# SunJiamei/LRP-ImageCaptioning

Measured on AMD Instinct MI355X. Metric: LRP heatmaps/sec (per predicted token) VGG16+adaptive-attn, 224x224, higher is better.
Workload: dtype bf16x3; 1 GPU; batch=32 synthetic 224x224 per GPU, VGG16 + adaptive-attention, LRP per-token heat-maps, 10 words/caption, V=10000 (BASELINE configs[1]); parallelism=image-sharded x1, RCCL weight broadcast, reverse_walk_precision=bf16x3, handles_per_gpu=2

## Files before the change

include/lrp_hip.h:

```cpp
#ifndef LRP_HIP_H
#define LRP_HIP_H

#include <stddef.h>
#include <stdint.h>

#ifdef __cplusplus
extern "C" {
#endif

#define LRP_ABI_VERSION 8

enum {
  LRP_OK = 0,
  LRP_ERR_INVALID = -1,
  LRP_ERR_STATE = -2,
  LRP_ERR_HIP = -3,
  LRP_ERR_NOMEM = -4,
  LRP_ERR_RANGE = -5,
  LRP_ERR_UNSUPPORTED = -6
};

enum { LRP_DEC_ADAPTIVE = 0,
       LRP_DEC_GRIDTD = 1 };

enum { LRP_EXPLAIN_SEQUENCE = 0,
       LRP_EXPLAIN_SINGLE_STEP = 1  };

enum { LRP_ENC_VGG = 0, LRP_ENC_RESNET = 1 };

#define LRP_MAX_CONV 32

typedef struct lrp_config {
  int32_t abi_version;
// ... 50 lines not shown

int lrp_decoder_gen_begin(lrp_handle* h, int32_t B, void* stream);
int lrp_decoder_gen_step(lrp_handle* h, int32_t B, const int32_t* parent_host, const int32_t* word_host, int32_t step,
                         double* logits_dev, void* stream);
int lrp_op_log_softmax_topk(const double* logits_dev, int32_t rows, int32_t V, int32_t k, int32_t* ids_dev,
                            double* logp_dev, void* stream);

int lrp_decoder_gradient(lrp_handle* h, int32_t n, const int32_t* img_idx_host, const int32_t* t_host,
                         float* d_feat_dev, double* r_words_dev, void* stream);
enum { LRP_WALK_LRP = 0, LRP_WALK_GRADIENT = 1, LRP_WALK_INPUT_X_GRADIENT = 2, LRP_WALK_GUIDED_BACKPROP = 3 };
int lrp_cnn_walk(lrp_handle* h, int32_t n, const int32_t* img_idx_host, const float* head_dev, float* out_dev,
                 int32_t walk, void* stream);

enum { LRP_PREC_FP32 = 0, LRP_PREC_BF16X3 = 1, LRP_PREC_BF16X3_FAST = 2, LRP_PREC_F16X2 = 3 };
int lrp_set_precision(lrp_handle* h, int32_t mode);
int lrp_set_fast_layers(lrp_handle* h, int64_t mask);

int lrp_profile_enable(lrp_handle* h, int32_t on);
int lrp_profile_query(lrp_handle* h, int64_t* n_launches, double* total_ms, double* total_flop);
int lrp_profile_records(lrp_handle* h, int32_t cap, double* ms_out, double* flop_out, int32_t* n_out);

int64_t lrp_workspace_bytes(const lrp_handle* h);

enum { LRP_CONV_SPLIT_BF16 = 0x100 };
int lrp_op_conv(const float* in_dev, const float* w_hwio_host, const float* bias_host,
                const float* aux_dev, float* out_dev, int32_t NB, int32_t H, int32_t W,
                int32_t Cin, int32_t Cout, int32_t taps, int32_t mode, void* stream);

int lrp_op_conv_pool_sparse(const float* sc_dev, const unsigned char* pos_dev, const float* w_hwio_host, const float* gate_dev,
                            float* out_dev, int32_t NB, int32_t Hp, int32_t Wp, int32_t Cin, int32_t Cout, int32_t reps, void* stream);

int lrp_op_epsilon_dense(const float* x_dev, const float* W_host, const float* R_dev, float* out_dev,
                         int32_t N, int32_t Din, int32_t Dout, float epsilon, void* stream);
int lrp_op_batchnorm_lrp(const float* x_dev, const float* gamma_dev, const float* beta_dev, const float* mean_dev,
                         const float* var_dev, float bn_eps, const float* R_dev, float* out_dev, int64_t n,
                         int32_t C, void* stream);
int lrp_op_add_lrp(const float* a_dev, const float* b_dev, const float* R_dev, float* Ra_dev, float* Rb_dev,
                   int64_t n, void* stream);

int lrp_op_avgpool_lrp(const float* x_dev, const float* R_dev, float* out_dev, int32_t NB, int32_t H, int32_t W,
                       int32_t C, int32_t k, void* stream);

int lrp_heatmap_render(const float* R_img_dev, const float* lut_dev, float* rgb_dev, int32_t n, int32_t npix, int32_t C,
                       float gamma, void* stream);

int lrp_preprocess_images(const uint8_t* rgb_dev, float* out_dev, int32_t NB, int32_t H0, int32_t W0, int32_t H,
                          int32_t W, void* stream);
// ... 57 lines not shown
```

lrp-imagecaptioning_amd/_capi.py:

```python
import ctypes as C
import os

HERE = os.path.dirname(os.path.abspath(__file__))
LIB_PATH = os.path.join(HERE, "liblrp_hip.so")

LRP_ABI_VERSION = 8
LRP_OK, LRP_ERR_INVALID, LRP_ERR_STATE, LRP_ERR_HIP, LRP_ERR_NOMEM, LRP_ERR_RANGE, LRP_ERR_UNSUPPORTED = 0, -1, -2, -3, -4, -5, -6
LRP_DEC_ADAPTIVE, LRP_DEC_GRIDTD = 0, 1
LRP_ENC_VGG, LRP_ENC_RESNET = 0, 1
LRP_EXPLAIN_SEQUENCE, LRP_EXPLAIN_SINGLE_STEP = 0, 1
LRP_PREC_FP32, LRP_PREC_BF16X3, LRP_PREC_BF16X3_FAST, LRP_PREC_F16X2 = 0, 1, 2, 3
LRP_MAX_CONV = 32
LRP_TRAIN_FP32, LRP_TRAIN_BF16 = 0, 1
LRP_EPI_BIAS_RELU, LRP_EPI_BIAS, LRP_EPI_MUL, LRP_EPI_MUL_UP2, LRP_EPI_FWD_DUAL, LRP_EPI_STORE, LRP_EPI_IMG_STENCIL = range(7)
LRP_OPND_FP32, LRP_OPND_BF16X3, LRP_OPND_F16X2 = 0, 1, 2
LRP_FORM_PLAIN, LRP_FORM_SMALL, LRP_FORM_HALO, LRP_FORM_BREG, LRP_FORM_POOL, LRP_FORM_IMG = range(6)
LRP_PLAN_FRAG, LRP_PLAN_JOIN, LRP_PLAN_DUAL_IL, LRP_PLAN_GMASK, LRP_PLAN_UP2_SRC, LRP_PLAN_IMG_PART, LRP_PLAN_POOL_GC = 1, 2, 4, 8, 16, 32, 64


class LrpConfig(C.Structure):
    _fields_ = [
        ("abi_version", C.c_int32), ("device", C.c_int32), ("decoder", C.c_int32),
        ("img_h", C.c_int32), ("img_w", C.c_int32), ("n_conv", C.c_int32),
        ("conv_cin", C.c_int32 * LRP_MAX_CONV), ("conv_cout", C.c_int32 * LRP_MAX_CONV),
        ("conv_pool_after", C.c_int32 * LRP_MAX_CONV), ("conv_name", (C.c_char * 32) * LRP_MAX_CONV),
        ("L", C.c_int32), ("D", C.c_int32), ("H", C.c_int32), ("E", C.c_int32), ("V", C.c_int32),
        ("max_images", C.c_int32), ("max_tokens", C.c_int32), ("max_caption_len", C.c_int32),
        ("sos_id", C.c_int32), ("eos_id", C.c_int32),
        ("encoder", C.c_int32), ("resnet_stem", C.c_int32), ("resnet_n_stacks", C.c_int32),
# ... 99 lines not shown
```

lrp-imagecaptioning_amd/csrc/conv_igemm.h:

```cpp
#pragma once
#include <hip/hip_runtime.h>
#include <stdint.h>
#include <stdlib.h>
#include <string.h>
#include <algorithm>
#include <vector>

#include "common.h"

namespace lrp {

typedef float f32x4 __attribute__((ext_vector_type(4)));
typedef float f32x16 __attribute__((ext_vector_type(16)));
typedef unsigned int u32x4 __attribute__((ext_vector_type(4)));
typedef __bf16 bf16x8 __attribute__((ext_vector_type(8)));
typedef _Float16 f16x8 __attribute__((ext_vector_type(8)));

enum ConvPrec { PREC_FP32 = 0, PREC_BF16X3 = 1, PREC_F16X2 = 2 };

__device__ __forceinline__ void split8h_store(const float* r, float* dst) {
  f16x8 hi, lo;
#pragma unroll
  for (int q = 0; q < 8; ++q) {
    hi[q] = (_Float16)r[q];
// ... 40 lines not shown
  ~TileOrder() {
    if (dev) (void)hipFree(dev);
    if (pinned) (void)hipHostFree(pinned);
    if (ev) (void)hipEventDestroy(ev);
  }
};

struct ConvArgs {
  const float* in;
  const float* wpk;
  const float* wpk_frag;
  int NB, H, W, Cin, CinP;
  int N;
  int taps;
  int M;
  int m_tiles, n_tiles;
  const float* bias;
  float* out;
  float* out2;
  const float* aux;
  const int* row2img;
  int split;
  int out_plain;
  int tiles_x, tiles_y, img_mode;
  const float* ximg;
  const float* addend;
  const float* gate_src;
  const float* join;
  const float* join_gate;
  const float* gate2;
  float* out2s;
  int gate_binary, relu_out;
  int dual_norelu;
  int dual_il, dual_gate;
  const float* bn_gamma; const float* bn_beta; const float* bn_mean; const float* bn_var;
  float bn_eps; int bn_relu;
  int tw, th, hrows, cols_t, nyh;
  const int* tile_map;
  TileOrder* order;
  const int* row2img_host;
  const float* tok_fac;
  unsigned* tok_max_out;
  const float* in_unscale;
  unsigned* act_max_out;
  float* pairs_out;
  const float* pairs_scale;
// ... 794 lines not shown
        for (int c = 0; c < 3; ++c) { pos[c] *= sc; neg[c] *= sc; }
      }
      const float* xv = a.ximg + ((size_t)img * HW + (size_t)y * a.W + x) * 3;
      float* ov = a.out + ((size_t)pn * HW + (size_t)y * a.W + x) * 3;
#pragma unroll
      for (int c = 0; c < 3; ++c) {
        if (a.img_mode == 0) ov[c] = xv[c] >= 0.f ? xv[c] * pos[c] : xv[c] * neg[c];
        else if (a.img_mode == 1) ov[c] = pos[c] + neg[c];
        else ov[c] = xv[c] * (pos[c] + neg[c]);
      }
    }
    return;
  } else if constexpr (EPI != EPI_STORE) {
    constexpr int NH = (BM * BN + 2 * STAGE - 1) / (2 * STAGE);
    constexpr int RH = BM / NH;
    static_assert(BM % NH == 0 && RH % (TM * 32) == 0 && RH * BN <= 2 * STAGE, "slab must hold whole wave tiles");
    float* Cs = smem;
    constexpr bool SPLIT_OUT = SPLIT && (EPI == EPI_MUL || EPI == EPI_MUL_UP2);
    constexpr int CW = SPLIT_OUT ? 8 : 4;
    constexpr int C4 = BN / CW, RPP = NT / C4;
    const int c4 = tid % C4, rin = tid / C4;
    const int col = n0 + c4 * CW;
    const int tn0 = m0 / HW, tp0 = m0 - tn0 * HW;
    const float invw = 1.0f / (float)a.W;
    auto locate = [&](int lr, int& row, int& n, int& h, int& w) -> bool {
      if constexpr (HALO) {
        int ty, tx;
        divmod(lr, a.tw, inv_tw, ty, tx);
        const int Y = Y0 + ty;
        w = x0 + tx;
        if (lr >= a.th * a.tw || Y >= yend || w >= a.W) return false;
        divmod(Y, a.H, inv_H, n, h);
        row = Y * a.W + w;
        return true;
      } else {
        row = m0 + lr;
        if (row >= a.M) return false;
        if constexpr (EPI == EPI_MUL || EPI == EPI_MUL_UP2) {
          n = tn0;
          int pix = tp0 + lr;
          while (pix >= HW) { pix -= HW; ++n; }
          h = (int)(((float)pix + 0.5f) * invw);
          w = pix - h * a.W;
          if (w < 0) { --h; w += a.W; } else if (w >= a.W) { ++h; w -= a.W; }
        }
        return true;
// ... 307 lines not shown
                }
              };
#pragma unroll
              for (int ps = 0; ps < RING - 1; ++ps) issue(ps);
              const bool plain = SPLIT_OUT && a.out_plain;
#pragma unroll
              for (int ps = 0; ps < NPf; ++ps) {
                if (ps + RING - 1 < NPf) issue(ps + RING - 1);
                int row, n_, h_, w_;
                if (locate(hf * RH + rin + ps * RPP, row, n_, h_, w_)) {
                  const int ll = rin + ps * RPP;
                  float v[CW];
#pragma unroll
                  for (int q4 = 0; q4 < CW / 4; ++q4)
                    *reinterpret_cast<f32x4*>(v + 4 * q4) = *reinterpret_cast<const f32x4*>(Cs + ll * BN + c4 * CW + 4 * q4);
#pragma unroll
                  for (int q = 0; q < UPf; ++q) {
                    float r[CW];
#pragma unroll
                    for (int q4 = 0; q4 < CW / 4; ++q4)
#pragma unroll
                      for (int e = 0; e < 4; ++e) r[4 * q4 + e] = v[4 * q4 + e] * gq[ps % RING][q][q4][e];
                    float* dst = EPI == EPI_MUL
                                     ? a.out + (size_t)row * a.N + col
                                     : a.out + (((size_t)n_ * H2f + 2 * h_ + (q >> 1)) * W2f + 2 * w_ + (q & 1)) * a.N + col;
                    if constexpr (SPLIT_OUT) {
                      if (plain) {
                        *reinterpret_cast<f32x4*>(dst) = *reinterpret_cast<const f32x4*>(r);
                        *reinterpret_cast<f32x4*>(dst + 4) = *reinterpret_cast<const f32x4*>(r + 4);
                      } else {
                        split8_store(r, dst);
                      }
                    } else {
                      *reinterpret_cast<f32x4*>(dst) = *reinterpret_cast<const f32x4*>(r);
                    }
                  }
                }
              }
              continue;
            }
          }
          constexpr int NP = RH / RPP;
          constexpr int UPN = EPI == EPI_MUL_UP2 ? 4 : 1;
          const int W2 = 2 * a.W, H2 = 2 * a.H;
          int rowv[NP], nv[NP], hv[NP], wv[NP], imgv[NP];
          bool okv[NP];
#pragma unroll
// ... 73 lines not shown
                *reinterpret_cast<f32x4*>(v + 4 * q4) = *reinterpret_cast<const f32x4*>(Cs + ll * BN + c4 * CW + 4 * q4);
#pragma unroll
              for (int q = 0; q < UPN; ++q) {
                float r[CW];
#pragma unroll
                for (int q4 = 0; q4 < CW / 4; ++q4) {
                  f32x4 g = cur.g[q][q4];
                  if (a.gate_binary) {
#pragma unroll
                    for (int e = 0; e < 4; ++e) g[e] = g[e] != 0.f ? 1.f : 0.f;
                  }
#pragma unroll
                  for (int e = 0; e < 4; ++e) {
                    float pr = v[4 * q4 + e] * g[e];
                    if (tail) pr += cur.jn[q4][e] * cur.jg[q4][e];
                    if constexpr (PREC == PREC_F16X2) {
                      pr *= fac16;
                      lmax = max(lmax, __float_as_uint(fabsf(pr)));
                    }
                    r[4 * q4 + e] = a.relu_out ? fmaxf(pr, 0.f) : pr;
                  }
                }
                float* dst = EPI == EPI_MUL
                                 ? a.out + (size_t)rowv[ps] * a.N + col
                                 : a.out + (((size_t)nv[ps] * H2 + 2 * hv[ps] + (q >> 1)) * W2 + 2 * wv[ps] + (q & 1)) * a.N + col;
                if constexpr (SPLIT_OUT) {
                  if (a.out_plain) {
                    *reinterpret_cast<f32x4*>(dst) = *reinterpret_cast<const f32x4*>(r);
                    *reinterpret_cast<f32x4*>(dst + 4) = *reinterpret_cast<const f32x4*>(r + 4);
                  } else if constexpr (PREC == PREC_F16X2) {
                    split8h_store(r, dst);
                  } else {
                    split8_store(r, dst);
                  }
                } else {
                  *reinterpret_cast<f32x4*>(dst) = *reinterpret_cast<const f32x4*>(r);
                }
                if (head2) {
                  float r2[CW];
#pragma unroll
                  for (int q4 = 0; q4 < CW / 4; ++q4)
#pragma unroll
                    for (int e = 0; e < 4; ++e) r2[4 * q4 + e] = r[4 * q4 + e] * cur.g2[q4][e];
                  float* d2 = a.out2s + (size_t)rowv[ps] * a.N + col;
                  if constexpr (SPLIT_OUT) {
                    split8_store(r2, d2);
                  } else {
// ... 258 lines not shown
  a.epi_generic = p.epi_generic;
}

template <int PREC>
inline hipError_t conv_launch_img(ConvArgs a, hipStream_t st) {
  if (!a.ximg || (PREC == PREC_F16X2 && !a.tok_fac)) return hipErrorInvalidValue;
  const ConvPlan p = conv_plan(conv_ask(EPI_IMG_STENCIL, PREC, 7, false, a));
  if (!p.ok) return hipErrorInvalidValue;
  if (a.NB <= 0) return hipSuccess;
  conv_apply_plan(p, a);
  a.tiles_x = (a.W + IMG_TILE - 1) / IMG_TILE;
  a.tiles_y = (a.H + IMG_TILE - 1) / IMG_TILE;
  hipLaunchKernelGGL((conv_igemm_kernel<4, 1, 2, 2, EPI_IMG_STENCIL, PREC>), dim3(a.m_tiles), dim3(p.threads), 0, st, a);
  return hipGetLastError();
}

template <int EPI, int PREC, int TERMS = 7, bool GMASK = false>
inline hipError_t conv_launch_epi(ConvArgs a, hipStream_t st) {
  static_assert(!GMASK || (EPI == EPI_MUL && PREC == PREC_FP32), "byte-mask gates: exact fp32 EPI_MUL only");
  constexpr bool MUL = EPI == EPI_MUL || EPI == EPI_MUL_UP2, FWD = EPI == EPI_BIAS || EPI == EPI_BIAS_RELU || EPI == EPI_FWD_DUAL;
  if (GMASK && (a.out2s || a.gate_none)) return hipErrorInvalidValue;
  if (PREC == PREC_F16X2 && MUL && (!a.tok_fac || !a.tok_max_out || a.out_plain)) return hipErrorInvalidValue;
  if (PREC == PREC_F16X2 && FWD && !a.in_unscale) return hipErrorInvalidValue;
  const ConvPlan p = conv_plan(conv_ask(EPI, PREC, TERMS, GMASK, a));
  if (!p.ok) return hipErrorInvalidValue;
  if (p.M <= 0 || a.N <= 0) return hipSuccess;
  if (a.pool_gc && (!a.pairs_out || !a.pool_pos)) return hipErrorInvalidValue;
  if (a.img_part && !a.img_w) return hipErrorInvalidValue;
  if (a.up2_src && (!a.up2_pairs || !a.up2_gpos)) return hipErrorInvalidValue;
  conv_apply_plan(p, a);
  const dim3 grid(p.m_tiles * p.n_tiles), block(p.threads);
  if constexpr (PREC != PREC_FP32 && (MUL || FWD)) {
    if (p.form == FORM_BREG || p.form == FORM_HALO || p.form == FORM_POOL) {
      if constexpr (MUL) {
        a.tile_map = conv_tile_order(a, st);
        if (p.form == FORM_BREG) {
          hipLaunchKernelGGL((conv_igemm_kernel<2, 2, 2, 1, EPI, PREC, true, true, TERMS>), grid, block, 0, st, a);
          return hipGetLastError();
        }
      }
      if (p.BM == 256)
        hipLaunchKernelGGL((conv_igemm_kernel<2, 4, 4, 2, EPI, PREC, true, false, TERMS>), grid, block, 0, st, a);
      else if (p.BN == 128)
        hipLaunchKernelGGL((conv_igemm_kernel<2, 2, 2, 2, EPI, PREC, true, false, TERMS>), grid, block, 0, st, a);
      else
        hipLaunchKernelGGL((conv_igemm_kernel<2, 2, 2, 1, EPI, PREC, true, false, TERMS>), grid, block, 0, st, a);
// ... 73 lines not shown
```

lrp-imagecaptioning_amd/csrc/conv_sparse.h:

```cpp
#pragma once
#include "cnn_kernels.h"
#include "conv_igemm.h"

namespace lrp {

typedef __bf16 bf16x16 __attribute__((ext_vector_type(16)));
typedef unsigned u32x2 __attribute__((ext_vector_type(2)));

struct SparseArgs {
  const float* sc;
  const unsigned* idxp;
  const float* wsp;
  const float* gate;
  float* out;
  const int* row2img;
  int NB, Hp, Wp, C, N;
  int cols_t, m_tiles, n_tiles;
  int out_plain;
  int diag;
};

constexpr int SP_TW = 14, SP_PITCH = SP_TW + 2;
constexpr int SP_BPACK = 32768, SP_NSTAGE = 4;

// ... 55 lines not shown
      const unsigned mh = px ^ qxm, mv = py ^ qym;
      const unsigned nmh = mh ^ 0x01010101u, nmv = mv ^ 0x01010101u;
      word[0][d] = P | ((P ^ 0x01010101u) << 2);
      word[1][d] = py | nmh | (nmh << 1);
      word[2][d] = (0x02020202u | ((mh & mv) ^ 0x01010101u)) << 2;
      word[3][d] = (px & mv) | (nmv << 1) | 0x0C0C0C0Cu;
    }
    unsigned h0[4], h1[4];
#pragma unroll
    for (int pl = 0; pl < 4; ++pl) {
      const unsigned t0 = word[pl][0] | (word[pl][0] >> 4), t1 = word[pl][1] | (word[pl][1] >> 4);
      h0[pl] = (t0 & 0xFFu) | (((t0 >> 16) & 0xFFu) << 8);
      h1[pl] = (t1 & 0xFFu) | (((t1 >> 16) & 0xFFu) << 8);
    }
    const u32x4 iw = {h0[0] | (h0[1] << 16), h0[2] | (h0[3] << 16), h1[0] | (h1[1] << 16), h1[2] | (h1[3] << 16)};
    const int spw = C >> 3;
    const size_t win = set / spw;
    const int sw = (int)(set - win * spw), chunk = sw >> 1, s2 = sw & 1;
    const size_t img = win / HW, pix = win - img * HW;
    reinterpret_cast<u32x4*>(idxp)[((((img * 4 + q) * (C >> 4) + chunk) * HW + pix) << 1) + s2] = iw;
  }
}

__global__ __launch_bounds__(256) void conv_sparse_pairs_kernel(const float* __restrict__ sc, float* __restrict__ scp, size_t n_sets, int HW, int C) {
  for (size_t i = (size_t)blockIdx.x * 256 + threadIdx.x; i < n_sets; i += (size_t)gridDim.x * 256) {
    float v[8];
    *reinterpret_cast<f32x4*>(v) = *reinterpret_cast<const f32x4*>(sc + i * 8);
    *reinterpret_cast<f32x4*>(v + 4) = *reinterpret_cast<const f32x4*>(sc + i * 8 + 4);
    const int spw = C >> 3;
    const size_t win = i / spw;
    const int sw = (int)(i - win * spw), chunk = sw >> 1, s2 = sw & 1;
    const size_t n = win / HW, pix = win - n * HW;
    split8_store(v, scp + ((((n * (C >> 4) + chunk) * HW + pix) << 1) + s2) * 8);
  }
}

__global__ __launch_bounds__(256) void conv_sparse_relayout_kernel(const float* __restrict__ pairs, float* __restrict__ scp, size_t n_sets, int HW, int C) {
  for (size_t i = (size_t)blockIdx.x * 256 + threadIdx.x; i < n_sets; i += (size_t)gridDim.x * 256) {
    const u32x4 hi = *reinterpret_cast<const u32x4*>(pairs + i * 8), lo = *reinterpret_cast<const u32x4*>(pairs + i * 8 + 4);
    const int spw = C >> 3;
    const size_t win = i / spw;
    const int sw_ = (int)(i - win * spw), chunk = sw_ >> 1, s2 = sw_ & 1;
    const size_t n = win / HW, pix = win - n * HW;
    float* dst = scp + ((((n * (C >> 4) + chunk) * HW + pix) << 1) + s2) * 8;
    *reinterpret_cast<u32x4*>(dst) = hi;
    *reinterpret_cast<u32x4*>(dst + 4) = lo;
  }
}

__global__ __launch_bounds__(256) void conv_sparse_pack_kernel(const float* __restrict__ wb, float* __restrict__ wsp, int N, int C, int CPo,
                                                               int n_tiles) {
  const size_t total = (size_t)4 * n_tiles * (C / 16) * 6 * 2 * 2 * 256;
  for (size_t i = (size_t)blockIdx.x * 256 + threadIdx.x; i < total; i += (size_t)gridDim.x * 256) {
    const int col = (int)(i & 255);
    size_t r = i >> 8;
    const int part = (int)(r & 1); r >>= 1;
    const int half = (int)(r & 1); r >>= 1;
    const int step = (int)(r % 6); r /= 6;
    const int chunk = (int)(r % (C / 16)); r /= (C / 16);
    const int nt = (int)(r % n_tiles);
    const int q = (int)(r / n_tiles);
    const int ci = nt * 256 + col;
    bf16x8 hi, lo;
#pragma unroll
    for (int e = 0; e < 8; ++e) {
      const int k32 = 16 * half + 8 * part + e, cb = k32 >> 2, slot = k32 & 3;
      const int ch8 = 4 * ((cb >> 1) & 1) + 2 * (cb >> 2) + (cb & 1);
// ... 77 lines not shown
    int n_, wy;
    divmod(Ys >= 0 && Ys < nys ? Ys : 0, Hp, inv_Hp, n_, wy);
    imgtab[tid] = a.row2img ? a.row2img[n_] : n_;
  }
  const __amdgpu_buffer_rsrc_t rsS = __builtin_amdgcn_make_buffer_rsrc((void*)a.sc, 0, 0x7FFFFFFF, RSRC_FLAGS);
  const __amdgpu_buffer_rsrc_t rsI = __builtin_amdgcn_make_buffer_rsrc((void*)a.idxp, 0, 0x7FFFFFFF, RSRC_FLAGS);
  constexpr int OOB = (int)0x80000000;
  auto fire_a = [&](int slot, int set8, int abuf) {
    int wv = wave_s, ln = lane;
    asm volatile("" : "+s"(wv), "+v"(ln));
    int pj = wv + NW * slot;
    if (pj >= TL::APIECES) pj = TL::APIECES - 1;
    const int pl = pj / TL::SUBPIECES, jp = pj - pl * TL::SUBPIECES;
    const int first = jp * 64 < PENT - 64 ? jp * 64 : PENT - 64;
    const int e = first + ln;
    const int hy = e >> 4, hx = e & 15;
    const int Ys = Y0 - 1 + hy, wx = x0 - 1 + hx;
    const bool ok = e < NENT && Ys >= 0 && Ys < nys && wx >= 0 && wx < Wp;
    int n_, wy;
    divmod(ok ? Ys : 0, Hp, inv_Hp, n_, wy);
    const int chunk = set8 >> 1, s = set8 & 1;
    int vo;
    if (pl < 2) {
      vo = ((((n_ * (C >> 4) + chunk) * Hp + wy) * Wp + wx) << 6) + s * 32 + pl * 16;
    } else {
      const int img = imgtab[ok ? hy : 0];
      vo = (((((img * 4 + q) * (C >> 4) + chunk) * Hp + wy) * Wp + wx) << 5) + s * 16;
    }
    __builtin_amdgcn_raw_ptr_buffer_load_lds(pl < 2 ? rsS : rsI, (lptr_t)(As + abuf * ABUF + pl * SUB + first * 16), 16, ok ? vo : OOB,
                                             0, 0, 0);
  };
  auto fire_set = [&](int set8, int abuf) {
#pragma unroll
    for (int sl = 0; sl < TL::ASLOTS; ++sl) fire_a(sl, set8, abuf);
  };

  const int nsteps2 = nchunks * 6;
  auto bsrc = [&](int chunk, int t6) { return chunk * 6 + 2 * (t6 % 3) + t6 / 3; };
  __syncthreads();
  fire_set(0, 0);
  if (nchunks * 2 > 1) fire_set(1, 1);
  fire_b(bsrc(0, 0), 0);
  fire_b(bsrc(0, 1), 1);
  asm volatile("s_waitcnt vmcnt(0)" ::: "memory");
  __syncthreads();

  f32x16 acc[MI][NJ];
// ... 131 lines not shown
    }
  }
#endif
}

inline size_t conv_sparse_weight_floats(int N, int C) { return (size_t)4 * ((N + 255) / 256) * (C / 16) * 6 * (SP_BPACK / 4); }
inline bool conv_sparse_supports(int N, int C, int Hp, int Wp) { return N % 256 == 0 && C % 16 == 0 && Hp >= 1 && Wp >= 1; }

inline hipError_t conv_sparse_pack(const float* wb_dev, float* wsp_dev, int N, int C, hipStream_t st) {
  const int n_tiles = (N + 255) / 256;
  const size_t total = (size_t)4 * n_tiles * (C / 16) * 6 * 2 * 2 * 256;
  hipLaunchKernelGGL(conv_sparse_pack_kernel, dim3((unsigned)((total + 255) / 256)), dim3(256), 0, st, wb_dev, wsp_dev, N, C, conv_cinp(C), n_tiles);
  return hipGetLastError();
}

inline size_t conv_sparse_index_words(int images, int Hp, int Wp, int C) { return (size_t)images * Hp * Wp * (C / 8) * 4 * 4; }
inline hipError_t conv_sparse_index(const unsigned char* pos_dev, unsigned* idxp_dev, int images, int Hp, int Wp, int C, hipStream_t st) {
  const size_t n_sets = (size_t)images * Hp * Wp * (C / 8);
  hipLaunchKernelGGL(conv_sparse_index_kernel, dim3(stream_grid(n_sets * 4)), dim3(256), 0, st, pos_dev, idxp_dev, n_sets, Hp * Wp, C);
  return hipGetLastError();
}
inline hipError_t conv_sparse_pairs(const float* sc_dev, float* scp_dev, int NB, int Hp, int Wp, int C, hipStream_t st) {
  const size_t n_sets = (size_t)NB * Hp * Wp * (C / 8);
  hipLaunchKernelGGL(conv_sparse_pairs_kernel, dim3(stream_grid(n_sets)), dim3(256), 0, st, sc_dev, scp_dev, n_sets, Hp * Wp, C);
  return hipGetLastError();
}

constexpr long CONV_SPARSE_SMALL_BLOCKS = 96L;
inline long conv_sparse_large_blocks(int NB, int Hp, int Wp, int N) {
  return 4L * ((NB * Hp + SparseTileLarge::TH - 1) / SparseTileLarge::TH) * ((Wp + SP_TW - 1) / SP_TW) * (N / SparseTileLarge::BN);
}
inline bool conv_sparse_small_grid(int NB, int Hp, int Wp, int N) {
  return sw().conv_small != 0 && conv_sparse_large_blocks(NB, Hp, Wp, N) <= CONV_SPARSE_SMALL_BLOCKS;
}

template <class TL>
inline hipError_t conv_sparse_launch_tile(SparseArgs a, hipStream_t st) {
  a.cols_t = (a.Wp + SP_TW - 1) / SP_TW;
  a.n_tiles = a.N / TL::BN;
  a.m_tiles = ((a.NB * a.Hp + TL::TH - 1) / TL::TH) * a.cols_t;
  hipLaunchKernelGGL(conv_sparse_kernel<TL>, dim3(4 * a.m_tiles * a.n_tiles), dim3(TL::NT), 0, st, a);
  return hipGetLastError();
}

inline hipError_t conv_sparse_launch(SparseArgs a, hipStream_t st) {
  if (!conv_sparse_supports(a.N, a.C, a.Hp, a.Wp) || !a.sc || !a.idxp || !a.wsp || !a.gate || !a.out) return hipErrorInvalidValue;
  if (a.NB <= 0) return hipSuccess;
// ... 6 lines not shown
```

lrp-imagecaptioning_amd/csrc/encoder.h:

```cpp
#pragma once
#include <algorithm>
#include <functional>
#include <memory>
#include <string>
#include <vector>

#include "cnn_kernels.h"
#include "common.h"
#include "conv_igemm.h"
#include "conv_sparse.h"
#include "f16_operand.h"

namespace lrp {

struct ConvLayer {
  std::string name;
  int cin = 0, cout = 0, H = 0, W = 0;
  bool pool_after = false;
  bool have_w = false, have_b = false;
  DevBuf w_fwd;
  DevBuf w_fwd_a;
  DevBuf w_fwd_zs;
  DevBuf w_fwd_as;
  DevBuf w_fwd_h;
// ... 105 lines not shown
    const size_t B = (size_t)max_images, NT = (size_t)max_tokens;
    const size_t max_tok_act = std::max(max_act, (size_t)img_h * img_w * IMG_T_COLS);
    LRP_TRY(images.alloc(B * img_h * img_w * 3 * sizeof(float), total));
    LRP_TRY(a1.alloc(B * img_h * img_w * 64 * sizeof(float), total));
    LRP_TRY(bufX.alloc(B * max_act * sizeof(float), total));
    LRP_TRY(bufA.alloc(B * max_act * sizeof(float), total));
    LRP_TRY(bufZ.alloc(B * max_act * sizeof(float), total));
    LRP_TRY(bufXs.alloc(B * max_act * sizeof(float), total));
    LRP_TRY(bufXl.alloc(B * max_act * sizeof(float), total));
    LRP_TRY(feat.alloc(B * T.act_elems() * sizeof(float), total));
    LRP_TRY(ztop.alloc(B * T.act_elems() * sizeof(float), total));
    LRP_TRY(s0.alloc(NT * max_tok_act * sizeof(float), total));
    LRP_TRY(s1.alloc(NT * max_tok_act * sizeof(float), total));
    for (size_t i = 0; i + 1 < layers.size(); ++i) LRP_TRY(layers[i].G.alloc(B * layers[i].act_elems() * sizeof(float), total));
    for (size_t i = 0; i + 1 < layers.size(); ++i) {
      ConvLayer& Lc = layers[i];
      if (Lc.pool_after && conv_compact_shape(Lc.cin, Lc.cout, Lc.H, Lc.W)) {
        LRP_TRY(Lc.Gc.alloc(B * Lc.act_elems() / 4 * sizeof(float), total));
        LRP_TRY(Lc.Gpos.alloc(B * Lc.act_elems() / 4, total));
      }
    }
    for (size_t i = 0; i + 1 < layers.size(); ++i)
      if (layers[i].pool_after) LRP_TRY(layers[i].P.alloc(B * layers[i].act_elems() / 4 * sizeof(float), total));
    {
      size_t mx = 0;
      for (size_t i = 1; i + 1 < layers.size(); ++i) {
        ConvLayer& Lc = layers[i];
        if (!Lc.sparse_ok() || !Lc.Gpos.p || layers[i - 1].pool_after) continue;
        LRP_TRY(Lc.idxp.alloc(conv_sparse_index_words((int)B, Lc.H / 2, Lc.W / 2, Lc.cout) * sizeof(unsigned), total));
        mx = std::max(mx, NT * Lc.act_elems() / 4);
      }
      if (mx) LRP_TRY(sp_scp.alloc(mx * sizeof(float), total));
    }
    {
      int lo = 0, hi = 0;
      LRP_HIP_CHECK(hipDeviceGetStreamPriorityRange(&lo, &hi));
      LRP_HIP_CHECK(hipStreamCreateWithPriority(&side, hipStreamNonBlocking, lo));
    }
    LRP_HIP_CHECK(hipEventCreateWithFlags(&ev_fwd, hipEventDisableTiming));
    LRP_HIP_CHECK(hipEventCreateWithFlags(&ev_gates, hipEventDisableTiming));
    LRP_TRY(act_max.alloc((layers.size() + 1) * B * ACT_MAX_SLOTS * sizeof(unsigned), total));
    LRP_TRY(act_unscale.alloc((layers.size() + 1) * B * sizeof(float), total));
    LRP_TRY(out_scale.alloc((layers.size() + 1) * B * sizeof(float), total));
    for (ConvLayer& L : layers) LRP_TRY(L.fnorm.alloc(2 * sizeof(float), total));
    return LRP_OK;
  }

  bool keep_acts = false;
  int enable_keep_acts(int64_t* total) {
    if (keep_acts) return LRP_OK;
    for (size_t li = 0; li + 1 < layers.size(); ++li) {
      ConvLayer& L = layers[li];
      if (!L.pool_after) LRP_TRY(L.Akeep.alloc((size_t)max_images * L.act_elems() * sizeof(float), total));
    }
    keep_acts = true;
// ... 480 lines not shown
      const size_t per4 = T.act_elems() / 4;
      hipLaunchKernelGGL(top_divide_kernel, dim3(stream_grid((size_t)n * per4)), dim3(256), 0, st,
                         reinterpret_cast<const f32x4*>(R_feat_dev), ztop.as<f32x4>(), row2img_dev,
                         reinterpret_cast<f32x4*>(S), n, per4);
      LRP_HIP_CHECK(hipGetLastError());
    }
    const bool up2_on = sw().up2_compact != 0;
    bool pairs_in = false;
    const bool fold_on = sw().img_fold != 0 && split && !f16 && walk == 0 && !layer_hook && img_fused() && layers.size() > 1 &&
                         !layers[0].pool_after && layers[1].cin == 64 && layers[0].w_bwd_s.p != nullptr;
    auto walk_plan = [&](int lc, bool up2) {
      const ConvLayer& Lc = layers[lc];
      ConvAsk q;
      q.epi = layers[lc - 1].pool_after ? EPI_MUL_UP2 : EPI_MUL; q.prec = run_prec;
      q.NB = n; q.H = Lc.H; q.W = Lc.W; q.N = Lc.cin; q.Cin = Lc.cout; q.taps = 9;
      q.frag = split && walk == 0 && Lc.w_bwd_frag.p != nullptr;
      q.up2_src = up2; q.img_part = lc == 1 && fold_on;
      return conv_plan(q);
    };
    auto sparse_consumer = [&](int lc) {
      if (lc < 1) return false;
      const ConvLayer& Lc = layers[lc];
      return sw().sparse_pool && Lc.w_sp.p && Lc.idxp.p && Lc.idx_epoch == encode_epoch && !layers[lc - 1].pool_after && split && !f16 &&
             walk == 0 && !layer_hook && sp_scp.p != nullptr;
    };
    auto writes_pairs = [&](int li) {
      const ConvLayer& P = layers[li - 1];
      if (!P.pool_after || !split || f16 || walk != 0 || layer_hook || li < 2 || (P.cout & 7) || !P.Gc.p || P.gc_epoch != encode_epoch)
        return false;
      if (sparse_consumer(li - 1)) return true;
      return up2_on && walk_plan(li - 1, true).ok;
    };
    for (int li = (int)layers.size() - 1; li >= 0; --li) {
      const ConvLayer& L = layers[li];
      if (layer_hook) {
        LRP_TRY((*layer_hook)(li, S));
        if (li == 0) return LRP_OK;
      }
      ConvArgs ca{};
      ConvPlan fold{};
      ca.in = S; ca.NB = n; ca.H = L.H; ca.W = L.W; ca.Cin = L.cout; ca.CinP = conv_cinp(L.cout); ca.taps = 9;
      if (hook_split) {
        const size_t n8 = (size_t)n * L.act_elems() / 8;
        hipLaunchKernelGGL(split_copy_kernel, dim3(stream_grid(n8)), dim3(256), 0, st, S, bufXs.as<float>(), n8);
        LRP_HIP_CHECK(hipGetLastError());
        ca.in = bufXs.as<float>();
        ca.out_plain = 1;
      }
// ... 8 lines not shown
        ca.tok_fac = tok_fac.as<float>();
        if (li > 0) ca.tok_max_out = lev_max(li - 1);
      }
      ca.row2img = row2img_dev;
      ca.order = L.order.get(); ca.row2img_host = r2i_host;
      ca.gate_binary = walk != 0; ca.relu_out = walk == 3;
      int epi;
      if (li == 0 && img_fused()) {
        ca.taps = 1; ca.N = IMG_T_COLS; ca.out = R_img_dev; ca.ximg = images.as<float>();
        ca.img_mode = walk == 0 ? 0 : walk == 2 ? 2 : 1;
        epi = EPI_IMG_STENCIL;
      } else if (li == 0) {
        ca.NB = n * L.H * L.W; ca.H = 1; ca.W = 1; ca.taps = 1;
        ca.N = IMG_T_COLS; ca.out = Snext; epi = EPI_STORE;
      } else {
        const ConvLayer& P = layers[li - 1];
        ca.N = L.cin; ca.aux = P.G.as<float>(); ca.out = Snext;
        epi = P.pool_after ? EPI_MUL_UP2 : EPI_MUL;
        if (li == 1 && fold_on && (fold = walk_plan(1, pairs_in)).ok) {
          ca.img_w = P.w_bwd_s.as<float>(); ca.img_part = Snext; ca.out = nullptr;
        }
        if (pairs_in && sparse_consumer(li)) {
          const int Hp = L.H / 2, Wp = L.W / 2;
          const size_t n_sets = (size_t)n * Hp * Wp * (L.cout / 8);
          ProfileRec pr{};
          if (profile) { (void)hipEventCreate(&pr.e0); (void)hipEventCreate(&pr.e1); (void)hipEventRecord(pr.e0, st); }
          hipLaunchKernelGGL(conv_sparse_relayout_kernel, dim3(stream_grid(n_sets)), dim3(256), 0, st, S, sp_scp.as<float>(), n_sets, Hp * Wp, L.cout);
          LRP_HIP_CHECK(hipGetLastError());
          SparseArgs sa{};
          sa.sc = sp_scp.as<float>(); sa.idxp = L.idxp.as<unsigned>(); sa.wsp = L.w_sp.as<float>(); sa.gate = P.G.as<float>(); sa.out = Snext;
          sa.row2img = row2img_dev; sa.NB = n; sa.Hp = Hp; sa.Wp = Wp; sa.C = L.cout; sa.N = L.cin;
          LRP_HIP_CHECK(conv_sparse_launch(sa, st));
          if (profile) {
            (void)hipEventRecord(pr.e1, st);
            pr.flop = 2.0 * (double)n * L.H * L.W * 9.0 * L.cout * L.cin;
            prof.push_back(pr);
          }
          pairs_in = false;
          float* t = S; S = Snext; Snext = t;
          continue;
        }
        if (pairs_in) {
          ca.up2_src = S; ca.up2_pairs = 1; ca.up2_gpos = L.Gpos.as<unsigned char>();
          pairs_in = false;
        }
        if (writes_pairs(li)) {
          epi = EPI_MUL; ca.aux = P.Gc.as<float>();
          pairs_in = true;
        }
      }
      ProfileRec pr{};
      if (profile) {
        (void)hipEventCreate(&pr.e0); (void)hipEventCreate(&pr.e1);
        (void)hipEventRecord(pr.e0, st);
      }
      const int terms = f16 && two_term(li) ? 5 : 7;
      if (epi == EPI_MUL_UP2) LRP_TRY(full_gate(li - 1, st));
      LRP_HIP_CHECK(conv_launch(epi, ca, st, run_prec, terms));
      if (profile) {
        (void)hipEventRecord(pr.e1, st);
        pr.flop = 2.0 * (double)n * L.H * L.W * 9.0 * L.cout * (li == 0 ? 6 : L.cin);
        prof.push_back(pr);
      }
      if (ca.img_part) {
        const ConvLayer& L0 = layers[0];
        ProfileRec p2{};
        if (profile) {
          (void)hipEventCreate(&p2.e0); (void)hipEventCreate(&p2.e1);
          (void)hipEventRecord(p2.e0, st);
        }
// ... 51 lines not shown
```

lrp-imagecaptioning_amd/csrc/engine.hip:

```cpp
#include <hip/hip_runtime.h>

#include <cmath>
#include <cstring>
#include <exception>
#include <map>
#include <new>
#include <string>
#include <vector>

#include "common.h"
#include "conv_igemm.h"
#include "conv_sparse.h"
#include "decoder.h"
#include "encoder.h"
#include "eval_kernels.h"
#include "resnet_encoder.h"
#include "rules_kernels.h"
#include "score_kernels.h"
#include "trainer.h"

namespace lrp {
std::string& last_error_ref() {
  static thread_local std::string e;
  return e;
// ... 396 lines not shown
}

static int op_pack_weight(const float* w_host, int taps, int Cin, int Cout, int bwd, DevBuf& raw, DevBuf& pk, hipStream_t st) {
  if (!raw.p) {
    LRP_TRY(raw.alloc((size_t)taps * Cin * Cout * sizeof(float), nullptr));
    LRP_HIP_CHECK(hipMemcpy(raw.p, w_host, raw.bytes, hipMemcpyHostToDevice));
  }
  const int rows = conv_npad(bwd ? Cin : Cout), CP = conv_cinp(bwd ? Cout : Cin);
  const size_t tot = (size_t)rows * taps * CP;
  LRP_TRY(pk.alloc(tot * sizeof(float), nullptr));
  hipLaunchKernelGGL(pack_conv_dev_kernel, dim3(stream_grid(tot)), dim3(256), 0, st, raw.as<float>(), pk.as<float>(), bwd, Cin, Cout, CP,
                     rows, 0, 0, taps);
  LRP_HIP_CHECK(hipGetLastError());
  return LRP_OK;
}

int lrp_op_conv(const float* in_dev, const float* w_hwio_host, const float* bias_host, const float* aux_dev, float* out_dev,
                int32_t NB, int32_t H, int32_t W, int32_t Cin, int32_t Cout, int32_t taps, int32_t mode, void* stream) {
  return guarded([&]() -> int {
    if (!in_dev || !w_hwio_host || !out_dev) return fail(LRP_ERR_INVALID, "null argument");
    if (taps != 1 && taps != 9) return fail(LRP_ERR_INVALID, "taps must be 1 or 9");
    if (Cin % 4 != 0) return fail(LRP_ERR_UNSUPPORTED, "Cin must be a multiple of 4");
    const bool split = (mode & LRP_CONV_SPLIT_BF16) != 0;
    mode &= ~LRP_CONV_SPLIT_BF16;
    if (mode < 0 || mode > 3) return fail(LRP_ERR_INVALID, "mode must be 0..3");
    if (split && mode == 0) return fail(LRP_ERR_UNSUPPORTED, "the split-bf16 path has no relu epilogue (modes 1..3)");
    const bool bwd = mode >= 2;
    const int inC = bwd ? Cout : Cin, outC = bwd ? Cin : Cout;
    if (inC % 4 != 0) return fail(LRP_ERR_UNSUPPORTED, "input channels must be a multiple of 4");
    if (split && ((inC & 7) || (bwd && (outC & 7)))) return fail(LRP_ERR_UNSUPPORTED, "split-bf16 path: channels must be multiples of 8");
    const int Np = conv_npad(outC), K = taps * conv_cinp(inC);
    hipStream_t st = S(stream);
    DevBuf wraw, wdev, wsplit, bdev, insplit, wfrag;
    LRP_TRY(op_pack_weight(w_hwio_host, taps, Cin, Cout, bwd, wraw, wdev, st));
    if (split) {
      const size_t nw8 = (size_t)Np * K / 8;
      LRP_TRY(wsplit.alloc(wdev.bytes, nullptr));
      hipLaunchKernelGGL(split_copy_kernel, dim3(stream_grid(nw8)), dim3(256), 0, st, wdev.as<float>(), wsplit.as<float>(), nw8);
      if (bwd && taps == 9 && Np == 64) {
        LRP_TRY(wfrag.alloc((size_t)64 * K * sizeof(float), nullptr));
        hipLaunchKernelGGL(pack_frag64_dev_kernel, dim3(stream_grid((size_t)conv_cinp(inC) / 32 * 9 * 512)), dim3(256), 0, st,
                           wsplit.as<float>(), wfrag.as<float>(), conv_cinp(inC));
      }
      const size_t n8 = (size_t)NB * H * W * inC / 8;
      LRP_TRY(insplit.alloc(n8 * 32, nullptr));
      hipLaunchKernelGGL(split_copy_kernel, dim3(stream_grid(n8)), dim3(256), 0, st, in_dev, insplit.as<float>(), n8);
      LRP_HIP_CHECK(hipGetLastError());
      in_dev = insplit.as<float>();
    }
    ConvArgs ca{};
    ca.out_plain = 1;
    ca.wpk_frag = wfrag.as<float>();
    ca.in = in_dev; ca.wpk = split ? wsplit.as<float>() : wdev.as<float>(); ca.NB = NB; ca.H = H; ca.W = W; ca.Cin = inC; ca.CinP = conv_cinp(inC);
    ca.N = outC; ca.taps = taps; ca.out = out_dev; ca.aux = aux_dev;
    if (!bwd) {
      if (!bias_host) return fail(LRP_ERR_INVALID, "bias required for forward modes");
      LRP_TRY(bdev.alloc((size_t)Cout * sizeof(float), nullptr));
      LRP_HIP_CHECK(hipMemcpy(bdev.p, bias_host, (size_t)Cout * sizeof(float), hipMemcpyHostToDevice));
      ca.bias = bdev.as<float>();
    } else if (!aux_dev) {
      return fail(LRP_ERR_INVALID, "aux (gate) required for backward modes");
    }
    static const int epi_of_mode[4] = {EPI_BIAS_RELU, EPI_BIAS, EPI_MUL, EPI_MUL_UP2};
    LRP_HIP_CHECK(conv_launch(epi_of_mode[mode], ca, st, split ? PREC_BF16X3 : PREC_FP32));
    LRP_HIP_CHECK(hipStreamSynchronize(st));
    return LRP_OK;
  });
}

int lrp_op_conv_pool_sparse(const float* sc_dev, const unsigned char* pos_dev, const float* w_hwio_host, const float* gate_dev,
                            float* out_dev, int32_t NB, int32_t Hp, int32_t Wp, int32_t Cin, int32_t Cout, int32_t reps, void* stream) {
  return guarded([&]() -> int {
    if (!sc_dev || !pos_dev || !w_hwio_host || !gate_dev || !out_dev) return fail(LRP_ERR_INVALID, "null argument");
    if (NB < 1 || Hp < 1 || Wp < 1 || (reps & 255) < 1) return fail(LRP_ERR_INVALID, "NB, Hp, Wp, reps must be >= 1");
// ... 360 lines not shown
```

lrp-imagecaptioning_amd/engine.py:

```python
import ctypes as C

import numpy as np
import torch

from . import _capi
from .synthetic import VGG16_CFG


def _i32(a):
    a = np.ascontiguousarray(np.asarray(a, dtype=np.int32))
    return a, a.ctypes.data_as(C.POINTER(C.c_int32))


class LRPEngine(object):

    def __init__(self, decoder="adaptive", cnn_cfg=VGG16_CFG, img_hw=(224, 224), L=196, D=512, H=512, E=512,
                 V=10000, max_images=32, max_tokens=320, max_caption_len=21, sos_id=2, eos_id=1, device=None,
                 resnet=None):
        if decoder not in ("adaptive", "gridtd"):
            raise NotImplementedError("decoder must be 'adaptive' or 'gridtd'")
        self._lib = _capi.load()
        if not torch.cuda.is_available():
            raise RuntimeError("LRPEngine needs a ROCm GPU (no CPU fallback for the LRP hot path)")
        self.device = torch.device("cuda", torch.cuda.current_device() if device is None else device)
# ... 333 lines not shown
            self.captions = None
        self.fast_layers = mask

    def profile_enable(self, on=True):
        _capi.check(self._lib.lrp_profile_enable(self._h, int(bool(on))))

    def profile_query(self):
        n, ms, fl = C.c_int64(), C.c_double(), C.c_double()
        _capi.check(self._lib.lrp_profile_query(self._h, C.byref(n), C.byref(ms), C.byref(fl)))
        return n.value, ms.value, fl.value


def _profile_records(self, cap=256):
    ms = (C.c_double * cap)()
    fl = (C.c_double * cap)()
    n = C.c_int32()
    _capi.check(self._lib.lrp_profile_records(self._h, cap, ms, fl, C.byref(n)))
    return [(ms[i], fl[i]) for i in range(n.value)]


LRPEngine.profile_records = _profile_records


CONV_SPLIT_BF16 = 0x100


def op_conv(x, w_hwio, bias, aux, mode, taps=9, split_bf16=False):
    lib = _capi.load()
    dev = x.device
    w = np.ascontiguousarray(w_hwio, dtype=np.float32)
    Cin, Cout = w.shape[2], w.shape[3]
    NB, H, W, _ = x.shape
    bwd = mode >= 2
    if mode == 3:
        out = torch.empty((NB, 2 * H, 2 * W, Cin), dtype=torch.float32, device=dev)
    elif bwd:
        out = torch.empty((NB, H, W, Cin), dtype=torch.float32, device=dev)
    else:
        out = torch.empty((NB, H, W, Cout), dtype=torch.float32, device=dev)
    b = np.ascontiguousarray(bias, dtype=np.float32) if bias is not None else None
    _capi.check(lib.lrp_op_conv(C.c_void_p(x.data_ptr()), w.ctypes.data_as(C.c_void_p),
                                b.ctypes.data_as(C.c_void_p) if b is not None else None,
                                C.c_void_p(aux.data_ptr()) if aux is not None else None,
                                C.c_void_p(out.data_ptr()), NB, H, W, Cin, Cout, taps,
                                mode | (CONV_SPLIT_BF16 if split_bf16 else 0),
                                C.c_void_p(torch.cuda.current_stream(dev).cuda_stream)))
    return out


def op_conv_pool_sparse(sc, pos, w_hwio, gate, reps=1):
    lib = _capi.load()
    w = np.ascontiguousarray(w_hwio, dtype=np.float32)
    Cin, Cout = w.shape[2], w.shape[3]
    NB, Hp, Wp, _ = sc.shape
    assert pos.dtype == torch.uint8 and tuple(pos.shape) == tuple(sc.shape) and tuple(gate.shape) == (NB, 2 * Hp, 2 * Wp, Cin)
    sc, pos, gate = sc.contiguous(), pos.contiguous(), gate.contiguous()
    out = torch.empty((NB, 2 * Hp, 2 * Wp, Cin), dtype=torch.float32, device=sc.device)
    _capi.check(lib.lrp_op_conv_pool_sparse(C.c_void_p(sc.data_ptr()), C.c_void_p(pos.data_ptr()), w.ctypes.data_as(C.c_void_p),
                                            C.c_void_p(gate.data_ptr()), C.c_void_p(out.data_ptr()), NB, Hp, Wp, Cin, Cout, int(reps),
                                            _cur_stream(sc.device)))
    return out


def op_sgemm(A, B, transA=False, transB=False, C_init=None, split=True):
    lib = _capi.load()
    M, K = (A.shape[1], A.shape[0]) if transA else A.shape
    N = B.shape[0] if transB else B.shape[1]
    out = torch.empty((M, N), dtype=torch.float32, device=A.device) if C_init is None else C_init
# ... 210 lines not shown
```

Baseline: 9929 heatmaps/s.

## Write conv backward output chunk-major so sparse pool consumer skips relayout

The EPI_MUL conv epilogue that feeds the sparse pooled conv can now store its bf16 pair output in a chunk-of-16-channels-major layout, the layout the sparse kernel reads. The sparse kernel's addressing and the pairs/relayout kernels change to that layout, so the separate relayout pass and its scratch buffer are no longer needed by default. The scratch buffer is now only allocated lazily on the fallback path. The cost is more scattered epilogue stores, which may lose some coalescing.

```diff
diff --git a/include/lrp_hip.h b/include/lrp_hip.h
--- a/include/lrp_hip.h
+++ b/include/lrp_hip.h
@@ -8,7 +8,7 @@
 extern "C" {
 #endif
 
-#define LRP_ABI_VERSION 8
+#define LRP_ABI_VERSION 9
 
 enum {
   LRP_OK = 0,
@@ -105,7 +105,7 @@
 
 int64_t lrp_workspace_bytes(const lrp_handle* h);
 
-enum { LRP_CONV_SPLIT_BF16 = 0x100 };
+enum { LRP_CONV_SPLIT_BF16 = 0x100, LRP_CONV_OUT_PAIRS = 0x200, LRP_CONV_OUT_CHUNK16 = 0x400 };
 int lrp_op_conv(const float* in_dev, const float* w_hwio_host, const float* bias_host,
                 const float* aux_dev, float* out_dev, int32_t NB, int32_t H, int32_t W,
                 int32_t Cin, int32_t Cout, int32_t taps, int32_t mode, void* stream);
diff --git a/lrp-imagecaptioning_amd/_capi.py b/lrp-imagecaptioning_amd/_capi.py
--- a/lrp-imagecaptioning_amd/_capi.py
+++ b/lrp-imagecaptioning_amd/_capi.py
@@ -4,7 +4,7 @@
 HERE = os.path.dirname(os.path.abspath(__file__))
 LIB_PATH = os.path.join(HERE, "liblrp_hip.so")
 
-LRP_ABI_VERSION = 8
+LRP_ABI_VERSION = 9
 LRP_OK, LRP_ERR_INVALID, LRP_ERR_STATE, LRP_ERR_HIP, LRP_ERR_NOMEM, LRP_ERR_RANGE, LRP_ERR_UNSUPPORTED = 0, -1, -2, -3, -4, -5, -6
 LRP_DEC_ADAPTIVE, LRP_DEC_GRIDTD = 0, 1
 LRP_ENC_VGG, LRP_ENC_RESNET = 0, 1
diff --git a/lrp-imagecaptioning_amd/csrc/conv_igemm.h b/lrp-imagecaptioning_amd/csrc/conv_igemm.h
--- a/lrp-imagecaptioning_amd/csrc/conv_igemm.h
+++ b/lrp-imagecaptioning_amd/csrc/conv_igemm.h
@@ -86,6 +86,7 @@
   const int* row2img;
   int split;
   int out_plain;
+  int out_chunk16;
   int tiles_x, tiles_y, img_mode;
   const float* ximg;
   const float* addend;
@@ -926,6 +927,9 @@
     const int c4 = tid % C4, rin = tid / C4;
     const int col = n0 + c4 * CW;
     const int tn0 = m0 / HW, tp0 = m0 - tn0 * HW;
+    const bool chunk16 = SPLIT_OUT && EPI == EPI_MUL && a.out_chunk16;
+    const int ost_row = chunk16 ? 16 : a.N;
+    const size_t ocol = chunk16 ? (size_t)(col >> 4) * a.M * 16 + (col & 8) : (size_t)col;
     const float invw = 1.0f / (float)a.W;
     auto locate = [&](int lr, int& row, int& n, int& h, int& w) -> bool {
       if constexpr (HALO) {
@@ -1279,7 +1283,7 @@
 #pragma unroll
                       for (int e = 0; e < 4; ++e) r[4 * q4 + e] = v[4 * q4 + e] * gq[ps % RING][q][q4][e];
                     float* dst = EPI == EPI_MUL
-                                     ? a.out + (size_t)row * a.N + col
+                                     ? a.out + (size_t)row * ost_row + ocol
                                      : a.out + (((size_t)n_ * H2f + 2 * h_ + (q >> 1)) * W2f + 2 * w_ + (q & 1)) * a.N + col;
                     if constexpr (SPLIT_OUT) {
                       if (plain) {
@@ -1399,7 +1403,7 @@
                   }
                 }
                 float* dst = EPI == EPI_MUL
-                                 ? a.out + (size_t)rowv[ps] * a.N + col
+                                 ? a.out + (size_t)rowv[ps] * ost_row + ocol
                                  : a.out + (((size_t)nv[ps] * H2 + 2 * hv[ps] + (q >> 1)) * W2 + 2 * wv[ps] + (q & 1)) * a.N + col;
                 if constexpr (SPLIT_OUT) {
                   if (a.out_plain) {
@@ -1704,6 +1708,7 @@
   if (GMASK && (a.out2s || a.gate_none)) return hipErrorInvalidValue;
   if (PREC == PREC_F16X2 && MUL && (!a.tok_fac || !a.tok_max_out || a.out_plain)) return hipErrorInvalidValue;
   if (PREC == PREC_F16X2 && FWD && !a.in_unscale) return hipErrorInvalidValue;
+  if (a.out_chunk16 && (EPI != EPI_MUL || PREC != PREC_BF16X3 || a.out_plain || (a.N & 15) || a.img_part || a.out2s)) return hipErrorInvalidValue;
   const ConvPlan p = conv_plan(conv_ask(EPI, PREC, TERMS, GMASK, a));
   if (!p.ok) return hipErrorInvalidValue;
   if (p.M <= 0 || a.N <= 0) return hipSuccess;
diff --git a/lrp-imagecaptioning_amd/csrc/conv_sparse.h b/lrp-imagecaptioning_amd/csrc/conv_sparse.h
--- a/lrp-imagecaptioning_amd/csrc/conv_sparse.h
+++ b/lrp-imagecaptioning_amd/csrc/conv_sparse.h
@@ -101,27 +101,25 @@
   }
 }
 
-__global__ __launch_bounds__(256) void conv_sparse_pairs_kernel(const float* __restrict__ sc, float* __restrict__ scp, size_t n_sets, int HW, int C) {
+__global__ __launch_bounds__(256) void conv_sparse_pairs_kernel(const float* __restrict__ sc, float* __restrict__ scp, size_t n_sets, int C) {
   for (size_t i = (size_t)blockIdx.x * 256 + threadIdx.x; i < n_sets; i += (size_t)gridDim.x * 256) {
     float v[8];
     *reinterpret_cast<f32x4*>(v) = *reinterpret_cast<const f32x4*>(sc + i * 8);
     *reinterpret_cast<f32x4*>(v + 4) = *reinterpret_cast<const f32x4*>(sc + i * 8 + 4);
     const int spw = C >> 3;
-    const size_t win = i / spw;
+    const size_t win = i / spw, n_win = n_sets / spw;
     const int sw = (int)(i - win * spw), chunk = sw >> 1, s2 = sw & 1;
-    const size_t n = win / HW, pix = win - n * HW;
-    split8_store(v, scp + ((((n * (C >> 4) + chunk) * HW + pix) << 1) + s2) * 8);
-  }
-}
-
-__global__ __launch_bounds__(256) void conv_sparse_relayout_kernel(const float* __restrict__ pairs, float* __restrict__ scp, size_t n_sets, int HW, int C) {
+    split8_store(v, scp + (((chunk * n_win + win) << 1) + s2) * 8);
+  }
+}
+
+__global__ __launch_bounds__(256) void conv_sparse_relayout_kernel(const float* __restrict__ pairs, float* __restrict__ scp, size_t n_sets, int C) {
   for (size_t i = (size_t)blockIdx.x * 256 + threadIdx.x; i < n_sets; i += (size_t)gridDim.x * 256) {
     const u32x4 hi = *reinterpret_cast<const u32x4*>(pairs + i * 8), lo = *reinterpret_cast<const u32x4*>(pairs + i * 8 + 4);
     const int spw = C >> 3;
-    const size_t win = i / spw;
+    const size_t win = i / spw, n_win = n_sets / spw;
     const int sw_ = (int)(i - win * spw), chunk = sw_ >> 1, s2 = sw_ & 1;
-    const size_t n = win / HW, pix = win - n * HW;
-    float* dst = scp + ((((n * (C >> 4) + chunk) * HW + pix) << 1) + s2) * 8;
+    float* dst = scp + (((chunk * n_win + win) << 1) + s2) * 8;
     *reinterpret_cast<u32x4*>(dst) = hi;
     *reinterpret_cast<u32x4*>(dst + 4) = lo;
   }
@@ -245,7 +243,7 @@
     const int chunk = set8 >> 1, s = set8 & 1;
     int vo;
     if (pl < 2) {
-      vo = ((((n_ * (C >> 4) + chunk) * Hp + wy) * Wp + wx) << 6) + s * 32 + pl * 16;
+      vo = ((((chunk * a.NB + n_) * Hp + wy) * Wp + wx) << 6) + s * 32 + pl * 16;
     } else {
       const int img = imgtab[ok ? hy : 0];
       vo = (((((img * 4 + q) * (C >> 4) + chunk) * Hp + wy) * Wp + wx) << 5) + s * 16;
@@ -423,7 +421,7 @@
 }
 inline hipError_t conv_sparse_pairs(const float* sc_dev, float* scp_dev, int NB, int Hp, int Wp, int C, hipStream_t st) {
   const size_t n_sets = (size_t)NB * Hp * Wp * (C / 8);
-  hipLaunchKernelGGL(conv_sparse_pairs_kernel, dim3(stream_grid(n_sets)), dim3(256), 0, st, sc_dev, scp_dev, n_sets, Hp * Wp, C);
+  hipLaunchKernelGGL(conv_sparse_pairs_kernel, dim3(stream_grid(n_sets)), dim3(256), 0, st, sc_dev, scp_dev, n_sets, C);
   return hipGetLastError();
 }
 
diff --git a/lrp-imagecaptioning_amd/csrc/encoder.h b/lrp-imagecaptioning_amd/csrc/encoder.h
--- a/lrp-imagecaptioning_amd/csrc/encoder.h
+++ b/lrp-imagecaptioning_amd/csrc/encoder.h
@@ -151,15 +151,10 @@
     }
     for (size_t i = 0; i + 1 < layers.size(); ++i)
       if (layers[i].pool_after) LRP_TRY(layers[i].P.alloc(B * layers[i].act_elems() / 4 * sizeof(float), total));
-    {
-      size_t mx = 0;
-      for (size_t i = 1; i + 1 < layers.size(); ++i) {
-        ConvLayer& Lc = layers[i];
-        if (!Lc.sparse_ok() || !Lc.Gpos.p || layers[i - 1].pool_after) continue;
-        LRP_TRY(Lc.idxp.alloc(conv_sparse_index_words((int)B, Lc.H / 2, Lc.W / 2, Lc.cout) * sizeof(unsigned), total));
-        mx = std::max(mx, NT * Lc.act_elems() / 4);
-      }
-      if (mx) LRP_TRY(sp_scp.alloc(mx * sizeof(float), total));
+    for (size_t i = 1; i + 1 < layers.size(); ++i) {
+      ConvLayer& Lc = layers[i];
+      if (!Lc.sparse_ok() || !Lc.Gpos.p || layers[i - 1].pool_after) continue;
+      LRP_TRY(Lc.idxp.alloc(conv_sparse_index_words((int)B, Lc.H / 2, Lc.W / 2, Lc.cout) * sizeof(unsigned), total));
     }
     {
       int lo = 0, hi = 0;
@@ -686,8 +681,9 @@
       if (lc < 1) return false;
       const ConvLayer& Lc = layers[lc];
       return sw().sparse_pool && Lc.w_sp.p && Lc.idxp.p && Lc.idx_epoch == encode_epoch && !layers[lc - 1].pool_after && split && !f16 &&
-             walk == 0 && !layer_hook && sp_scp.p != nullptr;
+             walk == 0 && !layer_hook;
     };
+    const bool sc_chunk = sw().sparse_pool != 2;
     auto writes_pairs = [&](int li) {
       const ConvLayer& P = layers[li - 1];
       if (!P.pool_after || !split || f16 || walk != 0 || layer_hook || li < 2 || (P.cout & 7) || !P.Gc.p || P.gc_epoch != encode_epoch)
@@ -742,13 +738,23 @@
         }
         if (pairs_in && sparse_consumer(li)) {
           const int Hp = L.H / 2, Wp = L.W / 2;
-          const size_t n_sets = (size_t)n * Hp * Wp * (L.cout / 8);
           ProfileRec pr{};
           if (profile) { (void)hipEventCreate(&pr.e0); (void)hipEventCreate(&pr.e1); (void)hipEventRecord(pr.e0, st); }
-          hipLaunchKernelGGL(conv_sparse_relayout_kernel, dim3(stream_grid(n_sets)), dim3(256), 0, st, S, sp_scp.as<float>(), n_sets, Hp * Wp, L.cout);
-          LRP_HIP_CHECK(hipGetLastError());
+          const float* sc = S;
+          if (!sc_chunk) {
+            if (!sp_scp.p) {
+              size_t mx = 0;
+              for (size_t i = 1; i + 1 < layers.size(); ++i)
+                if (layers[i].sparse_ok() && !layers[i - 1].pool_after) mx = std::max(mx, (size_t)max_tokens * layers[i].act_elems() / 4);
+              LRP_TRY(sp_scp.alloc(mx * sizeof(float), nullptr));
+            }
+            const size_t n_sets = (size_t)n * Hp * Wp * (L.cout / 8);
+            hipLaunchKernelGGL(conv_sparse_relayout_kernel, dim3(stream_grid(n_sets)), dim3(256), 0, st, S, sp_scp.as<float>(), n_sets, L.cout);
+            LRP_HIP_CHECK(hipGetLastError());
+            sc = sp_scp.as<float>();
+          }
           SparseArgs sa{};
-          sa.sc = sp_scp.as<float>(); sa.idxp = L.idxp.as<unsigned>(); sa.wsp = L.w_sp.as<float>(); sa.gate = P.G.as<float>(); sa.out = Snext;
+          sa.sc = sc; sa.idxp = L.idxp.as<unsigned>(); sa.wsp = L.w_sp.as<float>(); sa.gate = P.G.as<float>(); sa.out = Snext;
           sa.row2img = row2img_dev; sa.NB = n; sa.Hp = Hp; sa.Wp = Wp; sa.C = L.cout; sa.N = L.cin;
           LRP_HIP_CHECK(conv_sparse_launch(sa, st));
           if (profile) {
@@ -766,6 +772,7 @@
         }
         if (writes_pairs(li)) {
           epi = EPI_MUL; ca.aux = P.Gc.as<float>();
+          ca.out_chunk16 = sc_chunk && sparse_consumer(li - 1);
           pairs_in = true;
         }
       }
diff --git a/lrp-imagecaptioning_amd/csrc/engine.hip b/lrp-imagecaptioning_amd/csrc/engine.hip
--- a/lrp-imagecaptioning_amd/csrc/engine.hip
+++ b/lrp-imagecaptioning_amd/csrc/engine.hip
@@ -442,8 +442,11 @@
     if (taps != 1 && taps != 9) return fail(LRP_ERR_INVALID, "taps must be 1 or 9");
     if (Cin % 4 != 0) return fail(LRP_ERR_UNSUPPORTED, "Cin must be a multiple of 4");
     const bool split = (mode & LRP_CONV_SPLIT_BF16) != 0;
-    mode &= ~LRP_CONV_SPLIT_BF16;
+    const bool pairs_out = (mode & LRP_CONV_OUT_PAIRS) != 0, chunk16 = (mode & LRP_CONV_OUT_CHUNK16) != 0;
+    mode &= ~(LRP_CONV_SPLIT_BF16 | LRP_CONV_OUT_PAIRS | LRP_CONV_OUT_CHUNK16);
     if (mode < 0 || mode > 3) return fail(LRP_ERR_INVALID, "mode must be 0..3");
+    if ((pairs_out || chunk16) && !(split && mode == 2 && pairs_out && (!chunk16 || Cin % 16 == 0)))
+      return fail(LRP_ERR_UNSUPPORTED, "pairs output: mode 2 on the split-bf16 path only (chunk-major: with LRP_CONV_OUT_PAIRS, Cin %% 16 == 0)");
     if (split && mode == 0) return fail(LRP_ERR_UNSUPPORTED, "the split-bf16 path has no relu epilogue (modes 1..3)");
     const bool bwd = mode >= 2;
     const int inC = bwd ? Cout : Cin, outC = bwd ? Cin : Cout;
@@ -469,7 +472,7 @@
       in_dev = insplit.as<float>();
     }
     ConvArgs ca{};
-    ca.out_plain = 1;
+    ca.out_plain = pairs_out ? 0 : 1; ca.out_chunk16 = chunk16 ? 1 : 0;
     ca.wpk_frag = wfrag.as<float>();
     ca.in = in_dev; ca.wpk = split ? wsplit.as<float>() : wdev.as<float>(); ca.NB = NB; ca.H = H; ca.W = W; ca.Cin = inC; ca.CinP = conv_cinp(inC);
     ca.N = outC; ca.taps = taps; ca.out = out_dev; ca.aux = aux_dev;
diff --git a/lrp-imagecaptioning_amd/engine.py b/lrp-imagecaptioning_amd/engine.py
--- a/lrp-imagecaptioning_amd/engine.py
+++ b/lrp-imagecaptioning_amd/engine.py
@@ -379,10 +379,10 @@
 LRPEngine.profile_records = _profile_records
 
 
-CONV_SPLIT_BF16 = 0x100
-
-
-def op_conv(x, w_hwio, bias, aux, mode, taps=9, split_bf16=False):
+CONV_SPLIT_BF16, CONV_OUT_PAIRS, CONV_OUT_CHUNK16 = 0x100, 0x200, 0x400
+
+
+def op_conv(x, w_hwio, bias, aux, mode, taps=9, split_bf16=False, out_pairs=None):
     lib = _capi.load()
     dev = x.device
     w = np.ascontiguousarray(w_hwio, dtype=np.float32)
@@ -396,11 +396,12 @@
     else:
         out = torch.empty((NB, H, W, Cout), dtype=torch.float32, device=dev)
     b = np.ascontiguousarray(bias, dtype=np.float32) if bias is not None else None
+    flags = {None: 0, "window": CONV_OUT_PAIRS, "chunk16": CONV_OUT_PAIRS | CONV_OUT_CHUNK16}[out_pairs]
     _capi.check(lib.lrp_op_conv(C.c_void_p(x.data_ptr()), w.ctypes.data_as(C.c_void_p),
                                 b.ctypes.data_as(C.c_void_p) if b is not None else None,
                                 C.c_void_p(aux.data_ptr()) if aux is not None else None,
                                 C.c_void_p(out.data_ptr()), NB, H, W, Cin, Cout, taps,
-                                mode | (CONV_SPLIT_BF16 if split_bf16 else 0),
+                                mode | (CONV_SPLIT_BF16 if split_bf16 else 0) | flags,
                                 C.c_void_p(torch.cuda.current_stream(dev).cuda_stream)))
     return out
 
```

New measurement: 10010 heatmaps/s (median of 6 runs). No clear change (+0.8%).
